# amansanghvi/Thesis

Measured on AMD Instinct MI355X. Metric: particle-updates/sec (particles x scans/s) @1081 beams, higher is better.
Workload: dtype int8 map cells (lattice log-odds), f64 poses/weights; 1 GPU; BASELINE configs[2]: room16 synthetic, 4096 particles/GPU, 1081 beams, 0.05 m grid, K=30 samples, both matcher stages, resample every step; particles_per_gpu=4096, beams=1081, parallelism=particles sharded x1

## Files before the change

thesis_amd/csrc/kernels_match.hip:

```cpp
#include <limits.h>
#include <string.h>

#include <hip/hip_ext.h>

#include "rbpf_internal.h"
#include "rbpf_device.h"

namespace rbpf {

#ifdef RBPF_STAMPS
#define MSTAMP(k) do { if (tid == 0) { long long t_ = clock64(); st_acc[k] += t_ - st_prev; st_prev = t_; } } while (0)
#else
#define MSTAMP(k) do { } while (0)
#endif

static const int MBLOCK = 512;
static const int M_COARSE = 4;
static const int M_FINE_T = 4;
static const int M_FINE_R = 4;

struct MatchArgs {
    int mode;
    int single;
    const double* ref_xy; int n_ref;
    double guess[3]; double range[3];
    double* out;
    int N;
    int ds;
    double mcs;
    double d0;
    double rot_range;
    double max_range;
    const float* sel_x; const float* sel_y; int n_sel;
    int n_coarse_rot;
    int cap_sel;
    int sc_cap;
    double cell_off;
    int ndt;
    int ndt_nc;
    int ndt_max_iter;
    const int32_t* dup_of;
    uint32_t* ndt_occ;
    double* ndt_aux;
};

struct __attribute__((packed, aligned(4))) MaskPair { uint32_t lo, hi; };
struct __attribute__((packed, aligned(4))) MaskTriple { uint32_t w0, w1, w2; };

struct MatchLds {
    uint32_t* occ;
    uint32_t* dil;
    uint32_t* crs;
    float* fx4; float* fy4;
    float* cx8; float* cy8;
    int* sc;
};

__host__ __device__ inline int match_crs_words(int N) { return ((N / M_COARSE) + 15) / 16; }
static const int CRS_PAD = 7;
// ... 44 lines not shown
    double gx, gy, gth, rx, ry;
    if (a.single) {
        gx = a.guess[0]; gy = a.guess[1]; gth = a.guess[2]; rx = a.range[0]; ry = a.range[1];
    } else {
        gx = pose5[0]; gy = pose5[1]; gth = pose5[2];
        double c00 = pose5[3], c11 = pose5[4];
        double p0 = sqrt(c00) * 30.0, p1 = sqrt(c11) * 30.0;
        ry = fmax(fmin(4 * p1, 0.7), 0.1);
        rx = fmax(fmin(4 * p0, 0.7), 0.1);
    }
    g[0] = gx; g[1] = gy; g[2] = gth; rng[0] = rx; rng[1] = ry;
    org[0] = (int)floor(gx / a.mcs) - a.N / 2;
    org[1] = (int)floor(gy / a.mcs) - a.N / 2;
}

__device__ inline void match_frame(const DevView& v, const MatchArgs& a, int p, double* g, double* rng, int* org) {
    double pose5[5] = {0, 0, 0, 0, 0};
    if (!a.single) { pose5[0] = v.px[p]; pose5[1] = v.py[p]; pose5[2] = v.pth[p]; pose5[3] = v.cov[p]; pose5[4] = v.cov[(size_t)4 * v.P + p]; }
    match_frame_from(a, pose5, g, rng, org);
}

__global__ __launch_bounds__(MBLOCK) void match_kernel(DevView v, MatchArgs a) {
    extern __shared__ __align__(16) unsigned char smem[];
    const int N = a.N, W = N >> 5, tid = threadIdx.x, p = blockIdx.x;
    const int dup = a.dup_of ? a.dup_of[p] : p;
    double pre[5] = {0, 0, 0, 0, 0}; int pre_slot = 0;
    if (!a.single && tid == 0) { pre[0] = v.px[p]; pre[1] = v.py[p]; pre[2] = v.pth[p]; pre[3] = v.cov[p]; pre[4] = v.cov[(size_t)4 * v.P + p]; }
    if (!a.single) pre_slot = v.slot[p];
    if (dup != p) { if (tid == 0) atomicAdd(&v.stats[ST_MATCH_SHARED], 1ull); return; }
    MatchLds s;
    s.occ = reinterpret_cast<uint32_t*>(smem);
    s.dil = s.occ + (size_t)N * W;
    s.crs = s.dil + (size_t)N * W;
    const int cap4 = ((a.cap_sel + 3) / 4 + 7) & ~3, cap8 = ((a.cap_sel + 7) / 8 + 7) & ~3;
    s.fx4 = reinterpret_cast<float*>(s.crs + match_crs_total(N)); s.fy4 = s.fx4 + cap4;
    s.cx8 = s.fy4 + cap4; s.cy8 = s.cx8 + cap8;
    s.sc = reinterpret_cast<int*>(s.cy8 + cap8);
    __shared__ double s_g[3], s_rng[2];
    __shared__ int s_org[2], s_nb, s_best;
    __shared__ unsigned long long s_bestc;
    __shared__ unsigned s_def[32], s_slowg;
    __shared__ double s_mom[10], s_wmom[MBLOCK / 64][10];
    __shared__ int s_tab[49];

#ifdef RBPF_STAMPS
    long long st_acc[8] = {0, 0, 0, 0, 0, 0, 0, 0}, st_prev = clock64();
#endif
// ... 606 lines not shown
    const double A10 = m[5], A20 = m[6], A21 = m[8];
    if (!(A00 > 0)) return false;
    const double l00 = sqrt(A00), l10 = A10 / l00, l20 = A20 / l00;
    const double d1 = A11 - l10 * l10;
    if (!(d1 > 0)) return false;
    const double l11 = sqrt(d1), l21 = (A21 - l20 * l10) / l11;
    const double d2 = A22 - l20 * l20 - l21 * l21;
    if (!(d2 > 0)) return false;
    const double l22 = sqrt(d2);
    const double y0 = -m[1] / l00, y1 = (-m[2] - l10 * y0) / l11, y2 = (-m[3] - l20 * y0 - l21 * y1) / l22;
    d[2] = y2 / l22;
    d[1] = (y1 - l21 * d[2]) / l11;
    d[0] = (y0 - l10 * d[1] - l20 * d[2]) / l00;
    return true;
}

static const int NBLOCK = 256;
static const int NDT_STRIDE = 1;

size_t ndt_lds_bytes(int N, int B) { (void)B; return (size_t)(N + 2) * (N / 32 + 2) * 4 + 64; }

__global__ __launch_bounds__(NBLOCK, 4) void ndt_kernel(DevView v, MatchArgs a) {
    extern __shared__ __align__(16) unsigned char smem[];
    const int N = a.N, W = N >> 5, tid = threadIdx.x, p = blockIdx.x;
    uint32_t* occ = reinterpret_cast<uint32_t*>(smem);
    const float* __restrict__ bx = a.sel_x;
    const float* __restrict__ by = a.sel_y;
    const float inv = (float)(1.0 / a.mcs);
    __shared__ double s_g[3], s_rng[2], s_trial[6], s_w[NBLOCK / 64][10];
    __shared__ int s_org[2], s_go;
    __shared__ float s_lut[5][16];
    __shared__ unsigned s_ok;
#ifdef RBPF_STAMPS
    long long st_acc[8] = {0, 0, 0, 0, 0, 0, 0, 0}, st_prev = clock64();
#endif
    if (a.dup_of && a.dup_of[p] != p) return;
    const double* aux = a.ndt_aux + (size_t)p * 5;
    if (aux[4] == 0.0 || a.n_sel <= 0) return;
    if (tid == 0) { match_frame(v, a, p, s_g, s_rng, s_org); s_ok = 0; }
    const int WPD = W + 2;
    {
        const uint32_t* src = a.ndt_occ + (size_t)p * N * W;
        int u = tid / W, wv = tid % W;
        const int du = NBLOCK / W, dw = NBLOCK % W;
        const int SL = 16;
        for (int i0 = tid; i0 < N * W; i0 += SL * NBLOCK) {
            uint32_t val[SL]; int dst[SL];
// ... 164 lines not shown
    return (2 * n_coarse_rot + 1) * (2 * k + 1) * (2 * k + 1);
}
int match_per_rot(double max_range_m, double mcs) {
    int k = (int)ceil(max_range_m / mcs / M_COARSE);
    return (2 * k + 1) * (2 * k + 1);
}

__global__ void native_sincosf_kernel(const float* x, int n, float* s, float* c) {
    const int i = blockIdx.x * blockDim.x + threadIdx.x;
    if (i >= n) return;
    float sn, cs;
    __sincosf(x[i], &sn, &cs);
    s[i] = sn; c[i] = cs;
}
void launch_native_sincosf(const float* d_x, int n, float* d_s, float* d_c, hipStream_t s) {
    if (n > 0) hipLaunchKernelGGL(native_sincosf_kernel, dim3((n + 255) / 256), dim3(256), 0, s, d_x, n, d_s, d_c);
}

static void launch_match(const DevView& v, const MatchArgs& a_in, int grid, size_t lds, hipStream_t s, hipEvent_t t0 = nullptr, hipEvent_t t1 = nullptr) {
    MatchArgs a = a_in;
    a.sc_cap = match_sc_capacity(a.N, a.cap_sel, lds);
    static size_t lds_set[MAX_DEVICES] = {};
    ensure_dynamic_lds(reinterpret_cast<const void*>(match_kernel), lds, lds_set);
    if (t0 && t1) hipExtLaunchKernelGGL(match_kernel, dim3(grid), dim3(MBLOCK), lds, s, t0, t1, 0, v, a);
    else hipLaunchKernelGGL(match_kernel, dim3(grid), dim3(MBLOCK), lds, s, v, a);
}

int ndt_cells(double mcs) { return (int)floor(0.1 / mcs + 0.5); }

static void launch_ndt(const DevView& v, const MatchArgs& a, int grid, hipStream_t s, hipEvent_t t0 = nullptr, hipEvent_t t1 = nullptr) {
    size_t lds = ndt_lds_bytes(a.N, a.cap_sel);
    static size_t lds_set[MAX_DEVICES] = {};
    ensure_dynamic_lds(reinterpret_cast<const void*>(ndt_kernel), lds, lds_set);
    if (t0 && t1) hipExtLaunchKernelGGL(ndt_kernel, dim3(grid), dim3(NBLOCK), lds, s, t0, t1, 0, v, a);
    else hipLaunchKernelGGL(ndt_kernel, dim3(grid), dim3(NBLOCK), lds, s, v, a);
}

bool launch_match_particles(const DevView& v, int mode, const double* d_ref, int n_ref, double* d_out, int N, int ds,
                            double mcs, double d0, int ncr, double max_range, int cap_sel, size_t lds, int stage, hipStream_t s,
                            hipEvent_t t0, hipEvent_t t1) {
    MatchArgs a;
    memset(&a, 0, sizeof(a));
    a.mode = mode; a.single = 0; a.ref_xy = d_ref; a.n_ref = n_ref; a.out = d_out;
    a.N = N; a.ds = ds; a.mcs = mcs; a.d0 = d0; a.rot_range = 3.141592653589793 / 6; a.max_range = max_range;
    a.sel_x = mode ? v.asel_x : v.msel_x; a.sel_y = mode ? v.asel_y : v.msel_y; a.n_sel = mode ? v.n_asel : v.n_msel;
    a.n_coarse_rot = ncr; a.cap_sel = cap_sel;
    a.ndt = v.ndt_refine; a.ndt_nc = ndt_cells(mcs); a.ndt_max_iter = 500;
    a.dup_of = v.dups_valid ? v.dup_of : nullptr;
    const bool ndt = a.ndt && a.ndt_nc >= 2 && v.ndt_occ;
    if (ndt) { a.ndt_occ = v.ndt_occ; a.ndt_aux = v.ndt_aux; }
    if (stage == 1) launch_match(v, a, v.P, lds, s, t0, t1);
    if (stage == 2 && ndt) launch_ndt(v, a, v.P, s, t0, t1);
    return ndt;
}

void launch_match_single(const DevView& v, const double* d_ref, int n_ref, const double* guess3, const double* range3,
                         const float* d_sel_x, const float* d_sel_y, int n_sel, double* d_out, int N, int ds, double mcs,
                         double d0, int ncr, int cap_sel, size_t lds, uint32_t* d_ndt_occ, double* d_ndt_aux, hipStream_t s) {
    MatchArgs a;
    memset(&a, 0, sizeof(a));
    a.mode = 1; a.single = 1; a.ref_xy = d_ref; a.n_ref = n_ref; a.out = d_out;
    for (int i = 0; i < 3; ++i) { a.guess[i] = guess3[i]; a.range[i] = range3[i]; }
    a.N = N; a.ds = ds; a.mcs = mcs; a.d0 = d0; a.rot_range = range3[2]; a.max_range = 15.0;
    a.sel_x = d_sel_x; a.sel_y = d_sel_y; a.n_sel = n_sel; a.n_coarse_rot = ncr; a.cap_sel = cap_sel;
    a.cell_off = 0.5;
    a.ndt = v.ndt_refine; a.ndt_nc = ndt_cells(mcs); a.ndt_max_iter = 500;
    const bool ndt = a.ndt && a.ndt_nc >= 2 && d_ndt_occ;
    if (ndt) { a.ndt_occ = d_ndt_occ; a.ndt_aux = d_ndt_aux; }
    launch_match(v, a, 1, lds, s);
    if (ndt) launch_ndt(v, a, 1, s);
}

}
```

thesis_amd/csrc/kernels_propose.hip:

```cpp
#include "rbpf_internal.h"
#include "rbpf_device.h"

namespace rbpf {

#ifdef RBPF_STAMPS
#define PSTAMP(k) do { if (threadIdx.x == 0) { long long t_ = clock64(); atomicAdd(&v.stats[8 + (k)], (unsigned long long)(t_ - st_prev)); st_prev = t_; } } while (0)
#else
#define PSTAMP(k) do { } while (0)
#endif


static const int KMAX = 32;

__device__ __forceinline__ void philox_round(uint32_t c[4], uint32_t k0, uint32_t k1) {
    const uint64_t p0 = (uint64_t)0xD2511F53u * c[0], p1 = (uint64_t)0xCD9E8D57u * c[2];
    uint32_t n0 = (uint32_t)(p1 >> 32) ^ c[1] ^ k0, n1 = (uint32_t)p1;
    uint32_t n2 = (uint32_t)(p0 >> 32) ^ c[3] ^ k1, n3 = (uint32_t)p0;
    c[0] = n0; c[1] = n1; c[2] = n2; c[3] = n3;
}
__device__ void philox4x32(uint32_t ctr[4], uint64_t seed) {
    uint32_t k0 = (uint32_t)seed, k1 = (uint32_t)(seed >> 32);
#pragma unroll
    for (int r = 0; r < 10; ++r) { philox_round(ctr, k0, k1); k0 += 0x9E3779B9u; k1 += 0xBB67AE85u; }
}
// ... 27 lines not shown
                    double akp = a[k][p], akq = a[k][q];
                    a[k][p] = c * akp - s * akq; a[k][q] = s * akp + c * akq;
                }
                for (int k = 0; k < 3; ++k) {
                    double apk = a[p][k], aqk = a[q][k];
                    a[p][k] = c * apk - s * aqk; a[q][k] = s * apk + c * aqk;
                }
                for (int k = 0; k < 3; ++k) {
                    double vkp = V[k][p], vkq = V[k][q];
                    V[k][p] = c * vkp - s * vkq; V[k][q] = s * vkp + c * vkq;
                }
            }
    }
    for (int i = 0; i < 3; ++i) w[i] = a[i][i];
}

struct ProposeArgs {
    const double* match;
    const int32_t* match_of;
    const double* guesses;
    uint8_t* bad;
    uint64_t seed; uint32_t stream;
    double* dbg_w;
};


static const int PREP_W = 24;
__global__ __launch_bounds__(64) void propose_prep_kernel(DevView v, ProposeArgs a) {
    const int p = blockIdx.x * 64 + threadIdx.x;
    if (p >= v.P) return;
    const double* m = a.match + (size_t)(a.match_of ? a.match_of[p] : p) * 13;
    double* o = v.prop_prep + (size_t)p * PREP_W;
    bool bad = false;
    for (int i = 0; i < 9; ++i) bad |= isnan(m[3 + i]);
    a.bad[p] = bad ? 1 : 0;
    o[22] = bad ? 1.0 : 0.0;
    if (bad) return;
    double w[3], V[3][3];
    eig3_sym(m + 3, w, V);
    double mx = fmax(fabs(w[0]), fmax(fabs(w[1]), fabs(w[2])));
    double eps = 1e6 * 2.220446049250313e-16 * mx;
    double log_pdet = 0.0; int rank = 0;
    for (int j = 0; j < 3; ++j) {
        bool keep = w[j] > eps;
        if (!keep && fabs(w[j]) > eps) { a.bad[p] = 1; o[22] = 1.0; return; }
        double inv_sqrt = fabs(w[j]) > eps ? sqrt(1.0 / w[j]) : 0.0;
        if (keep) { log_pdet += log(w[j]); ++rank; }
        double sq = w[j] > 0 ? sqrt(w[j]) : 0.0;
        for (int i = 0; i < 3; ++i) { o[3 * i + j] = V[i][j] * inv_sqrt; o[9 + 3 * i + j] = V[i][j] * sq; }
    }
    o[18] = m[0]; o[19] = m[1]; o[20] = m[2];
    o[21] = -0.5 * ((double)rank * 1.8378770664093453 + log_pdet);
}

static const int SAMP_W = 256;
__global__ __launch_bounds__(256) void propose_samples_kernel(DevView v, ProposeArgs a) {
    const int gid = blockIdx.x * 256 + threadIdx.x, p = gid >> 5, k = gid & 31, K = v.K;
    if (p >= v.P || k >= K) return;
    const double* pr = v.prop_prep + (size_t)p * PREP_W;
    if (pr[22] != 0.0) return;
    const double mean[3] = {pr[18], pr[19], pr[20]};
    double g[3];
    if (a.guesses) {
        const double* gp = a.guesses + ((size_t)p * K + k) * 3;
        g[0] = gp[0]; g[1] = gp[1]; g[2] = gp[2];
    } else {
        double z[3];
        normals3(a.seed, a.stream, (uint32_t)v.global_id[p], (uint32_t)k, z);
        for (int i = 0; i < 3; ++i) g[i] = mean[i] + ((pr[9 + 3 * i] * z[0] + pr[9 + 3 * i + 1] * z[1]) + pr[9 + 3 * i + 2] * z[2]);
    }
    const double d0 = g[0] - mean[0], d1 = g[1] - mean[1], d2 = g[2] - mean[2];
    double maha = 0.0;
    for (int j = 0; j < 3; ++j) { double t = (d0 * pr[j] + d1 * pr[3 + j]) + d2 * pr[6 + j]; maha += t * t; }
    double sn, cs;
    sincos(g[2], &sn, &cs);
    int lx, ly, off_x = 0, off_y = 0;
    if (!(v.dim & 1) && tile_of_coord(mean[0], v.tile_len, v.R, lx) && tile_of_coord(mean[1], v.tile_len, v.R, ly)) {
        off_x = v.dim / 2 - lx * v.dim; off_y = v.dim / 2 - ly * v.dim;
    }
    const double inv_cs = (double)v.dim / v.tile_len;
    double* o = v.prop_samp + (size_t)p * SAMP_W;
// ... 98 lines not shown
    for (int i = tid; i < n_redo; i += BLOCK) {
        const uint32_t e = f.s_redo[i];
        const int b = (int)(e >> 5), kk = (int)(e & 31u);
        const double x = v.bx[b], y = v.by[b];
        const double gx = (s_c[kk] * x + (-s_s[kk]) * y) + s_g[kk][0];
        const double gy = (s_s[kk] * x + s_c[kk] * y) + s_g[kk][1];
        int vv;
        if (lookup_cell_home(v, home, s_tab, s_base, gx, gy, vv)) atomicAdd(&s_sum[kk], vv);
    }
    PSTAMP(3);
}

__global__ __launch_bounds__(BLOCK) void propose_weight_kernel(DevView v, ProposeArgs a) {
    __shared__ double s_c[KMAX], s_s[KMAX], s_g[KMAX][3], s_pr[KMAX], s_w[KMAX];
    __shared__ int s_sum[KMAX];
    __shared__ float4 s_q[KMAX];
    __shared__ int s_tab[49];
    __shared__ unsigned long long s_base[49];
    __shared__ double s_mean[3];
    __shared__ double s_mom[16];
    __shared__ int s_bad, s_nredo[2];
    __shared__ uint32_t s_redo[REDO_CAP];
    __shared__ __align__(16) float s_bx[WB_CAP], s_by[WB_CAP];
    const int p = blockIdx.x, tid = threadIdx.x, K = v.K;
    long long st_prev = clock64();
    if (tid == 0) { s_nredo[0] = 0; s_nredo[1] = 0; }
    const int LL = v.L * v.L;
    {
        const double* pr = v.prop_prep + (size_t)p * PREP_W;
        if (tid < 3) s_mean[tid] = pr[18 + tid];
        if (tid == 0) s_bad = pr[22] != 0.0;
    }
    const int32_t* tab = v.tile_tab + (size_t)v.slot[p] * LL;
    for (int i = tid; i < LL; i += BLOCK) {
        const int t = tab[i];
        s_tab[i] = t;
        s_base[i] = t >= 0 ? (unsigned long long)t * (unsigned long long)v.dim * (unsigned long long)v.dim : ~0ull;
    }
    __syncthreads();
    if (s_bad) {
        if (tid == 0) { v.upd_pose[p] = v.px[p]; v.upd_pose[v.P + p] = v.py[p]; v.upd_pose[2 * v.P + p] = v.pth[p]; }
        return;
    }
    const HomeTile home = home_tile(v, s_tab, s_mean[0], s_mean[1]);
    if (tid < K) {
        const double* sp = v.prop_samp + (size_t)p * SAMP_W;
        s_c[tid] = sp[tid]; s_s[tid] = sp[32 + tid]; s_g[tid][0] = sp[64 + tid]; s_g[tid][1] = sp[96 + tid]; s_g[tid][2] = sp[128 + tid];
// ... 81 lines not shown
        s_sum[tid] = 0;
    }
    __syncthreads();
    {
        const WeightFrame wf{s_c, s_s, s_g, s_q, s_sum, s_tab, s_base, s_redo, s_nredo, s_bx, s_by};
        weight_beams(v, home, wf, K, tid, st_prev);
    }
    __syncthreads();
    if (tid < K) {
        double obs = v.inv_quantum > 0 ? (v.inv_quantum + (double)s_sum[tid]) / v.inv_quantum : 1.0 + (double)s_sum[tid] * v.quantum;
        out_w[(size_t)p * K + tid] = obs * prs[(size_t)p * K + tid];
    }
}
void launch_weight_samples_product(const DevView& v, const double* d_guesses, const double* d_prs, int K, double* d_out_w, hipStream_t s) {
    hipLaunchKernelGGL(weight_samples_product_kernel, dim3(v.P), dim3(BLOCK), 0, s, v, d_guesses, d_prs, K, d_out_w);
}

__global__ __launch_bounds__(BLOCK) void bad_weight_kernel(DevView v, const uint8_t* __restrict__ bad) {
    if (!bad[blockIdx.x]) return;
    nan_branch_weight(v, blockIdx.x, threadIdx.x, BLOCK);
}

void launch_propose_weight(const DevView& v, const double* d_match, const int32_t* d_match_of, const double* d_guesses, uint8_t* d_bad,
                           uint64_t seed, uint32_t stream, double* d_dbg_w, hipStream_t s) {
    ProposeArgs a{d_match, d_match_of, d_guesses, d_bad, seed, stream, d_dbg_w};
    hipLaunchKernelGGL(propose_prep_kernel, dim3((v.P + 63) / 64), dim3(64), 0, s, v, a);
    hipLaunchKernelGGL(propose_samples_kernel, dim3((v.P * 32 + 255) / 256), dim3(256), 0, s, v, a);
    hipLaunchKernelGGL(propose_weight_kernel, dim3(v.P), dim3(BLOCK), 0, s, v, a);
}
void launch_bad_weight(const DevView& v, const uint8_t* d_bad, hipStream_t s) {
    hipLaunchKernelGGL(bad_weight_kernel, dim3(v.P), dim3(BLOCK), 0, s, v, d_bad);
}

}
```

thesis_amd/csrc/rbpf_api.hip:

```cpp
#include <math.h>
#include <stdio.h>
#include <stdlib.h>
#include <string.h>

#include <algorithm>
#include <initializer_list>
#include <limits>

#include "rbpf_host.h"
#include "rbpf_scanbatch.h"

using namespace rbpf;

static thread_local std::string g_create_err;

#define HIP_TRY(h, call)                                                                           \
    do {                                                                                           \
        hipError_t e_ = (call);                                                                    \
        if (e_ != hipSuccess) {                                                                    \
            (h)->err = std::string(#call) + ": " + hipGetErrorString(e_);                          \
            return RBPF_EDEVICE;                                                                   \
        }                                                                                          \
    } while (0)

// ... 33 lines not shown
    if (e != hipSuccess) { h->err = std::string("hipMalloc: ") + hipGetErrorString(e); return RBPF_ENOMEM; }
    *out = h->allocs.back().as<T>();
    return RBPF_OK;
}
#define ALLOC(h, ptr, n) do { int rc_ = dev_alloc(h, &(ptr), (n)); if (rc_) return rc_; } while (0)

static int check_device_error(rbpf_handle* h) {
    int32_t e = 0;
    HIP_TRY(h, hipMemcpyAsync(&e, h->v.err, sizeof(e), hipMemcpyDeviceToHost, h->stream));
    HIP_TRY(h, hipStreamSynchronize(h->stream));
    if (e != 0) {
        int32_t z = 0;
        hipMemcpyAsync(h->v.err, &z, sizeof(z), hipMemcpyHostToDevice, h->stream);
        hipStreamSynchronize(h->stream);
        const char* what = e == RBPF_ENOMEM ? "tile pool or work-item queue exhausted"
                         : e == RBPF_ERANGE ? "a pose or beam left the addressable tile lattice (raise lattice_radius)"
                         : "device-side error";
        return fail(h, e, what);
    }
    return RBPF_OK;
}

static bool env_is(const char* name, const char* value) { const char* e = getenv(name); return e && strcmp(e, value) == 0; }

static int track_take_place(rbpf_handle* h, bool implicit, int& t) {
    t = -1;
    if (h->track_n >= h->track_cap) {
        if (!implicit) return fail(h, RBPF_ENOMEM, "the trajectory log is full");
        h->track_dropped++;
        return RBPF_OK;
    }
    t = h->track_n++;
    return RBPF_OK;
}
static int track_queue(rbpf_handle* h, int t) {
    if (t < 0) return RBPF_OK;
    launch_track_record(h->v, h->track_log(), t, h->track_pending(h->track_cur), h->stream);
    HIP_TRY(h, hipGetLastError());
    return RBPF_OK;
}
static int track_record(rbpf_handle* h, bool implicit) {
    int t;
    const int rc = track_take_place(h, implicit, t);
    return rc ? rc : track_queue(h, t);
}

// ... 159 lines not shown
        ALLOC(h, v.prop_samp, 256 * P);
        ALLOC(h, v.stats, ST_COUNT); ALLOC(h, v.err, 1);
        ALLOC(h, v.mu_fallback, P); HIP_TRY(h, hipMemset(v.mu_fallback, 0, P * 4));
        ALLOC(h, v.ev_queue, 2); HIP_TRY(h, hipMemset(v.ev_queue, 0, 8));
        ALLOC(h, h->d_did_early, 1);
        HIP_TRY(h, hipMemset(h->d_did_early, 0, 4));
        HIP_TRY(h, h->events.create(&h->ev_weights, hipEventDisableTiming | hipEventDisableSystemFence));
        {
            v.mu_mode = env_is("RBPF_MAP_KERNEL", "window") ? MU_WINDOW : env_is("RBPF_MAP_KERNEL", "ray") ? MU_RAY : env_is("RBPF_MAP_KERNEL", "ev") ? MU_EV : MU_DEFAULT;
            v.ev_resident = env_is("RBPF_EV_RESIDENT", "0") ? 0 : 1;
            const char* eg = getenv("RBPF_EV_GRID");
            v.ev_grid = eg ? std::max(0, atoi(eg)) : 0;
            v.match_stage_slow = env_is("RBPF_MATCH_STAGE", "slow") ? 1 : 0;
            const char* ws = getenv("RBPF_WSAFE");
            v.wsafe_override = ws ? (float)atof(ws) : -1.0f;
            v.weight_entry_f64 = env_is("RBPF_WEIGHT_ENTRY", "f64") ? 1 : 0;
            v.ndt_refine = h->cfg.ndt_refine;
            h->dedup_enabled = !env_is("RBPF_MATCH_DEDUP", "0");
            {
                int cus = 0;
                if (hipDeviceGetAttribute(&cus, hipDeviceAttributeMultiprocessorCount, c.device) != hipSuccess || cus < 1) { (void)hipGetLastError(); cus = 1; }
                h->skip_discarded = !env_is("RBPF_SKIP_DISCARDED", "0");
                h->hold_back = getenv("RBPF_SKIP_DISCARDED") ? true : (long long)P > 4LL * cus;
            }
        }
        ALLOC(h, v.dup_of, P); v.dups_valid = 0;
        ALLOC(h, h->d_last_xy, 2 * (size_t)c.max_beams); ALLOC(h, h->d_tmp_sel, 2 * (size_t)c.max_beams);
        if (raycast_lds_bytes(c.max_beams, v.reach) > LDS_LIMIT) return fail(h, RBPF_EINVAL, "max_beams too large for the LDS window layout");
        match_geometry(c, c.cell_size, h->mN, h->mds, h->mmcs, h->md0, h->mncr);
        h->mlds = match_lds_bytes(h->mN, c.max_beams, match_max_coarse(h->mncr, 0.7, h->mmcs), match_per_rot(0.7, h->mmcs));
        if (h->mlds > LDS_LIMIT) return fail(h, RBPF_EINVAL, "matcher region does not fit in LDS for this cell_size");
        if (c.ndt_refine && ndt_cells(h->mmcs) >= 2) {
            if (ndt_lds_bytes(h->mN, c.max_beams) > LDS_LIMIT) return fail(h, RBPF_EINVAL, "NDT stage: matcher region does not fit in LDS");
            ALLOC(h, v.ndt_occ, P * (size_t)h->mN * (h->mN / 32)); ALLOC(h, v.ndt_aux, 5 * P);
        }
        ALLOC(h, h->d_match, 13 * P); ALLOC(h, h->d_bad, P); ALLOC(h, h->d_guess_full, P * (size_t)c.n_samples * 3);
        {
            ResampleBuffers& r = h->rs;
            ALLOC(h, r.T, P); ALLOC(h, r.idx, P); ALLOC(h, r.did, 1); ALLOC(h, r.slot2, P); ALLOC(h, r.dead_list, P);
            ALLOC(h, r.jobs, 2 * P); ALLOC(h, r.n_jobs, 2); ALLOC(h, r.pending_free, (size_t)v.pool_tiles); ALLOC(h, r.n_pending, 1);
            ALLOC(h, r.px2, P); ALLOC(h, r.py2, P); ALLOC(h, r.pth2, P); ALLOC(h, r.cov2, 9 * P); ALLOC(h, r.w2, P);
            ALLOC(h, r.skip, P); ALLOC(h, r.keep, P); ALLOC(h, r.plan, 2);
            HIP_TRY(h, hipMemset(r.n_pending, 0, 4)); HIP_TRY(h, hipMemset(r.n_jobs, 0, 8)); HIP_TRY(h, hipMemset(r.did, 0, 4));
            HIP_TRY(h, hipMemset(r.skip, 0, P)); HIP_TRY(h, hipMemset(r.plan, 0, 8));
        }
        HIP_TRY(h, hipMemset(v.pool, 0, (size_t)v.pool_tiles * cells));
// ... 6 lines not shown
        for (size_t p = 0; p < P; ++p) { ids[p] = (int32_t)p; tab[p * LL + (size_t)v.R * v.L + v.R] = (int32_t)p; }
        for (int t = 0; t < v.pool_tiles; ++t) { bb[4 * t] = INT32_MAX; bb[4 * t + 1] = -1; bb[4 * t + 2] = INT32_MAX; bb[4 * t + 3] = -1; }
        int32_t top = v.pool_tiles - (int32_t)P;
        for (int i = 0; i < top; ++i) fs[i] = v.pool_tiles - 1 - i;
        HIP_TRY(h, hipMemcpy(v.slot, ids.data(), P * 4, hipMemcpyHostToDevice));
        HIP_TRY(h, hipMemcpy(v.global_id, ids.data(), P * 4, hipMemcpyHostToDevice));
        HIP_TRY(h, hipMemcpy(v.tile_tab, tab.data(), P * LL * 4, hipMemcpyHostToDevice));
        HIP_TRY(h, hipMemcpy(v.free_stack, fs.data(), (size_t)v.pool_tiles * 4, hipMemcpyHostToDevice));
        HIP_TRY(h, hipMemcpy(v.free_top, &top, 4, hipMemcpyHostToDevice));
        HIP_TRY(h, hipMemcpy(v.tile_bbox, bb.data(), bb.size() * 4, hipMemcpyHostToDevice));
        return RBPF_OK;
    };
    rc = build();
    if (rc != RBPF_OK) { g_create_err = h->err; rbpf_destroy(h); return rc; }
    *out = h;
    return RBPF_OK;
}

int rbpf_destroy(rbpf_handle* h) {
    if (!h) return RBPF_OK;
    ON_DEVICE_HELD(h);
    h->mu_pending = false;
    if (hipStreamSynchronize(h->stream) != hipSuccess) (void)hipGetLastError();
    h->each_staging([](Staging& s) { if (s.wait() != hipSuccess) (void)hipGetLastError(); });
    if (h->ev_weights_valid && hipEventSynchronize(h->ev_weights) != hipSuccess) (void)hipGetLastError();
    for (Block& b : h->allocs) b.release();
    for (Block& b : h->buf) b.release();
    for (Block& b : h->track_mem) b.release();
    h->each_staging([](Staging& s) { s.release(); });
    h->each_staging([](Staging& s) { s.destroy_event(); });
    h->events.destroy();
    if (h->own_stream && h->stream) (void)hipStreamDestroy(h->stream);
    (void)hipGetLastError();
    delete h;
    return RBPF_OK;
}

const char* rbpf_last_error(const rbpf_handle* h) { return h ? h->err.c_str() : g_create_err.c_str(); }

int rbpf_set_stream(rbpf_handle* h, void* s) {
    if (!h) return RBPF_EINVAL;
    ON_DEVICE(h);
    HIP_TRY(h, hipStreamSynchronize(h->stream));
    if (h->own_stream && h->stream) (void)hipStreamDestroy(h->stream);
    h->own_stream = false;
    h->stream = static_cast<hipStream_t>(s);
    h->last_end = nullptr;
    return RBPF_OK;
}

int rbpf_release_stream(rbpf_handle* h) {
    if (!h) return RBPF_EINVAL;
    ON_DEVICE(h);
    if (h->own_stream) return RBPF_OK;
    HIP_TRY(h, hipStreamSynchronize(h->stream));
// ... 205 lines not shown
int rbpf_map_update(rbpf_handle* h, const double* poses) {
    if (!h) return RBPF_EINVAL;
    ON_DEVICE(h);
    h->v.dups_valid = 0;
    if (!h->have_scan) return fail(h, RBPF_ESTATE, "rbpf_set_scan has not been called");
    DevView& v = h->v;
    const size_t P = v.P;
    if (poses) {
        std::vector<double> soa(3 * P);
        for (size_t p = 0; p < P; ++p) { soa[p] = poses[3 * p]; soa[P + p] = poses[3 * p + 1]; soa[2 * P + p] = poses[3 * p + 2]; }
        HIP_TRY(h, hipMemcpyAsync(v.upd_pose, soa.data(), 3 * P * 8, hipMemcpyHostToDevice, h->stream));
        HIP_TRY(h, hipStreamSynchronize(h->stream));
    } else {
        HIP_TRY(h, hipMemcpyAsync(v.upd_pose, v.px, P * 8, hipMemcpyDeviceToDevice, h->stream));
        HIP_TRY(h, hipMemcpyAsync(v.upd_pose + P, v.py, P * 8, hipMemcpyDeviceToDevice, h->stream));
        HIP_TRY(h, hipMemcpyAsync(v.upd_pose + 2 * P, v.pth, P * 8, hipMemcpyDeviceToDevice, h->stream));
    }
    int rc = run_map_update(h, h->v);
    if (rc) return rc;
    h->scan_updates++;
    return check_device_error(h);
}

static int run_matcher(rbpf_handle* h, int32_t adj, const double* last_scan_xy, int32_t n_last) {
    DevView& v = h->v;
    if (adj && !last_scan_xy) {
        if (h->n_last_dev < 0) return fail(h, RBPF_ESTATE, "adj = 1 without last_scan_xy needs rbpf_refresh_last_scan first");
        n_last = h->n_last_dev;
    } else if (adj && (n_last < 0 || n_last > h->cfg.max_beams))
        return fail(h, RBPF_EINVAL, "adj = 1 needs last_scan_xy with at most max_beams points");
    if (adj && last_scan_xy) {
        void* slot = h->rings[R_LAST].acquire();
        memcpy(slot, last_scan_xy, (size_t)n_last * 16);
        HIP_TRY(h, hipMemcpyAsync(h->d_last_xy, slot, (size_t)n_last * 16, hipMemcpyHostToDevice, h->stream));
        h->rings[R_LAST].submitted(h->stream);
    }
    hipEvent_t t0 = nullptr, t1 = nullptr;
    h->prof_take(3, t0, t1);
    h->match_rows = v.dups_valid ? 2 : 1;
    const bool ndt = launch_match_particles(v, adj ? 1 : 0, h->d_last_xy, adj ? n_last : 0, h->d_match, h->mN, h->mds, h->mmcs, h->md0,
                                            h->mncr, h->cfg.match_max_range, h->cfg.max_beams, h->mlds, 1, h->stream, t0, t1);
    if (ndt) {
        h->prof_take(4, t0, t1);
        launch_match_particles(v, adj ? 1 : 0, h->d_last_xy, adj ? n_last : 0, h->d_match, h->mN, h->mds, h->mmcs, h->md0,
                               h->mncr, h->cfg.match_max_range, h->cfg.max_beams, h->mlds, 2, h->stream, t0, t1);
    }
    HIP_TRY(h, hipGetLastError());
    return RBPF_OK;
}

int rbpf_scan_update(rbpf_handle* h, int32_t adj, const double* last_scan_xy, int32_t n_last,
                     const double* match_override, const double* guesses) {
    int rc = rbpf_scan_update_begin(h, adj, last_scan_xy, n_last, match_override, guesses);
    if (rc || !h->map_updates || !h->hold_back) return rc ? rc : rbpf_scan_update_end(h);
    h->scan_begun = false;
    h->scan_updates++;
    h->mu_pending = true; h->mu_pending_rec = -1;
    if (h->track_on && (h->track_flags & RBPF_TRACK_SCAN)) return track_take_place(h, true, h->mu_pending_rec);
    return RBPF_OK;
}

int rbpf_scan_update_begin(rbpf_handle* h, int32_t adj, const double* last_scan_xy, int32_t n_last,
                           const double* match_override, const double* guesses) {
    if (!h) return RBPF_EINVAL;
    ON_DEVICE(h);
    if (!h->have_scan) return fail(h, RBPF_ESTATE, "rbpf_set_scan has not been called");
    DevView& v = h->v;
    const size_t P = v.P;
    if (match_override) {
        h->match_rows = 0;
        HIP_TRY(h, hipMemcpyAsync(h->d_match, match_override, 13 * P * 8, hipMemcpyHostToDevice, h->stream));
    } else {
        int rc = run_matcher(h, adj, last_scan_xy, n_last);
        if (rc) return rc;
    }
    const double* d_g = nullptr;
    if (guesses) {
        HIP_TRY(h, hipMemcpyAsync(h->d_guess_full, guesses, P * (size_t)v.K * 3 * 8, hipMemcpyHostToDevice, h->stream));
        d_g = h->d_guess_full;
    }
    if (!match_override && !guesses) h->prof_begin_chained(1); else h->prof_begin(1);
    const int32_t* match_of = (!match_override && v.dups_valid) ? v.dup_of : nullptr;
    if (h->prop_capture && !h->d_prop_w) ALLOC(h, h->d_prop_w, P * (size_t)v.K);
    launch_propose_weight(v, h->d_match, match_of, d_g, h->d_bad, h->cfg.seed, (uint32_t)h->scan_updates, h->prop_capture ? h->d_prop_w : nullptr, h->stream);
    h->prop_valid = true; h->prop_captured = h->prop_capture;
    v.dups_valid = 0;
    h->prof_end(1);
    HIP_TRY(h, hipGetLastError());
    h->ev_weights_valid = false;
    if (h->record_ev_weights) { HIP_TRY(h, hipEventRecord(h->ev_weights, h->stream)); h->ev_weights_valid = true; }
    h->scan_begun = true; h->begin_seen = true;
    return RBPF_OK;
}

int rbpf_scan_update_end(rbpf_handle* h) {
    if (!h) return RBPF_EINVAL;
    ON_DEVICE(h);
    if (!h->scan_begun) return fail(h, RBPF_ESTATE, "rbpf_scan_update_begin has not been called");
    h->scan_begun = false;
    if (!h->map_updates) {
        launch_bad_weight(h->v, h->d_bad, h->stream);
        HIP_TRY(h, hipGetLastError());
        h->scan_updates++;
    } else {
        const int rc = run_map_update(h, h->v, h->d_bad);
        if (rc) return rc;
        h->scan_updates++;
    }
    if (h->track_on && (h->track_flags & RBPF_TRACK_SCAN)) return track_record(h, true);
    return RBPF_OK;
// ... 2176 lines not shown
```

thesis_amd/csrc/rbpf_host.h:

```cpp
#pragma once
#include <stdlib.h>
#include <algorithm>
#include <string>
#include <vector>

#include "rbpf_internal.h"

static const size_t LDS_LIMIT = 160 * 1024;

enum MemKind { MEM_DEVICE, MEM_PINNED, MEM_PAGEABLE };
struct Block {
    MemKind kind = MEM_DEVICE;
    unsigned char* p = nullptr; size_t cap = 0;
    hipError_t reserve(size_t bytes) {
        if (p && cap >= bytes) return hipSuccess;
        release();
        const size_t want = kind == MEM_PINNED ? std::max<size_t>(bytes * 2, 1 << 16) : std::max<size_t>(bytes, 4096);
        hipError_t e = hipSuccess;
        if (kind == MEM_DEVICE) e = hipMalloc(reinterpret_cast<void**>(&p), want);
        else if (kind == MEM_PINNED) e = hipHostMalloc(reinterpret_cast<void**>(&p), want, hipHostMallocDefault);
        else if (!(p = static_cast<unsigned char*>(malloc(want)))) e = hipErrorOutOfMemory;
        if (e == hipSuccess) cap = want; else p = nullptr;
        return e;
    }
// ... 115 lines not shown
    hipError_t reserve(int b, size_t bytes) {
        if (buf[b].cap >= bytes) return hipSuccess;
        if (b >= B_DRAIN_FIRST) { const hipError_t e = hipStreamSynchronize(stream); if (e != hipSuccess) return e; }
        return buf[b].reserve(bytes);
    }
    PinnedRing rings[R_COUNT];
    EventPool events;
    template <typename F> void each_staging(F f) { for (Staging& s : stage) f(s); for (PinnedRing& r : rings) for (Staging& s : r.slot) f(s); }
    hipEvent_t ev_weights = nullptr; bool ev_weights_valid = false, record_ev_weights = false, begin_seen = false;
    int32_t* d_did_early = nullptr; bool scan_begun = false;
    int early_n = 0;
    unsigned char* d_scan = nullptr; size_t scan_bytes = 0;
    template <typename T> T* in_slot(unsigned char* slot, const T* dev) const { return reinterpret_cast<T*>(slot + (reinterpret_cast<const unsigned char*>(dev) - d_scan)); }
    int mN = 0, mds = 1, mncr = 0; double mmcs = 0, md0 = 0; size_t mlds = 0;
    double* d_last_xy = nullptr; float* d_tmp_sel = nullptr;
    int n_last_dev = -1;
    int match_rows = 0;
    double* d_match = nullptr; uint8_t* d_bad = nullptr; double* d_guess_full = nullptr;
    unsigned long long resample_draws = 0;
    int ev_workgroups = 0;
    bool map_updates = true;
    bool mu_pending = false; int mu_pending_rec = -1;
    bool hold_back = false, skip_discarded = true;
    static const int N_KERN = 5, RING = 512;
    std::vector<hipEvent_t> ring[N_KERN][2];
    int ring_n[N_KERN] = {0, 0, 0, 0, 0};
    std::vector<hipEvent_t> begin_used[N_KERN];
    hipEvent_t last_end = nullptr;
    bool timed(int k) const { return (prof_mask >> k) & 1u; }
    void prof_begin(int k) { if (!timed(k)) return; hipEvent_t e = ring[k][0][ring_n[k] % RING]; (void)hipEventRecord(e, stream); begin_used[k][ring_n[k] % RING] = e; if (k == 2) rs_split[ring_n[k] % RING] = 0; }
    void prof_begin_chained(int k) { if (!timed(k)) return; if (!last_end) { prof_begin(k); return; } begin_used[k][ring_n[k] % RING] = last_end; }
    void prof_end(int k) { if (!timed(k)) return; last_end = ring[k][1][ring_n[k] % RING]; (void)hipEventRecord(last_end, stream); ring_n[k]++; }
    std::vector<hipEvent_t> rs_mid[2]; std::vector<char> rs_split;
    void prof_pause(int k) { if (!timed(k)) return; const int slot = ring_n[k] % RING; (void)hipEventRecord(rs_mid[0][slot], stream); rs_split[slot] = 1; }
    void prof_resume(int k) { if (!timed(k)) return; (void)hipEventRecord(rs_mid[1][ring_n[k] % RING], stream); }
    hipError_t family_ms(int k, int slot, float* ms) {
        if (k != 2 || !rs_split[slot]) return hipEventElapsedTime(ms, begin_used[k][slot], ring[k][1][slot]);
        float a = 0, b = 0;
        hipError_t e = hipEventElapsedTime(&a, begin_used[k][slot], rs_mid[0][slot]);
        if (e == hipSuccess) e = hipEventElapsedTime(&b, rs_mid[1][slot], ring[k][1][slot]);
        *ms = a + b;
        return e;
    }
    bool prof_take(int k, hipEvent_t& t0, hipEvent_t& t1) {
        t0 = t1 = nullptr;
        if (!timed(k)) return false;
// ... 19 lines not shown
```

thesis_amd/csrc/rbpf_internal.h:

```cpp
#pragma once
#include <hip/hip_runtime.h>
#include <stdint.h>
#include <mutex>

#include "../../include/rbpf_hip.h"
#include "rbpf_math.h"
#include "rbpf_blockrelax.h"

namespace rbpf {

static const int MAX_DEVICES = 16;
inline void ensure_dynamic_lds(const void* fn, size_t bytes, size_t* set) {
    static std::mutex mu;
    std::lock_guard<std::mutex> lock(mu);
    int dev = 0;
    (void)hipGetDevice(&dev);
    const bool tracked = dev >= 0 && dev < MAX_DEVICES;
    if (tracked && bytes <= set[dev]) return;
    const hipError_t rc = hipFuncSetAttribute(fn, hipFuncAttributeMaxDynamicSharedMemorySize, (int)bytes);
    if (rc != hipSuccess) { (void)hipGetLastError(); return; }
    if (tracked) set[dev] = bytes;
}


// ... 323 lines not shown
void launch_readback(void* mapped_dst, const double* d_nan_elem, const int32_t* d_did, const int32_t* d_idx, int n, hipStream_t s);
bool map_update_ray_available(const DevView& v);
void launch_map_update_ray(const DevView& v, const int32_t* only, hipStream_t s, hipEvent_t t0 = nullptr, hipEvent_t t1 = nullptr);
bool map_update_ev_available(const DevView& v);
int launch_map_update_ev(const DevView& v, hipStream_t s, hipEvent_t t0 = nullptr, hipEvent_t t1 = nullptr);
void launch_get_odds(const DevView& v, int particle, const double* d_xy, int n, double* d_vals,
                     uint8_t* d_none, hipStream_t s);
void launch_last_scan(const DevView& v, int particle, double* d_out_xy, hipStream_t s);
void launch_imu_update(const DevView& v, int model, double d0, double d1, double d2, double dt_ticks,
                       const double* vel_noise, hipStream_t s);
void launch_resample_indices(int P, const double* d_w, double u, double spread, int32_t* d_T, int32_t* d_idx,
                             int32_t* d_did, int32_t* d_err, hipStream_t s);
void launch_resample_local(const DevView& v, const ResampleBuffers& b, const double* d_w, double u, double spread, hipStream_t s);
void launch_resample_plan_early(const DevView& v, const ResampleBuffers& b, const uint8_t* d_bad, int leave_out, double u, double spread, hipStream_t s);
void launch_resample_plan_late(const DevView& v, const ResampleBuffers& b, double u, double spread, hipStream_t s);
void launch_resample_copies(const DevView& v, const ResampleBuffers& b, hipStream_t s);
void launch_export_weights(const DevView& v, double* d_out, int n_global, const uint8_t* d_bad, hipStream_t s);
void launch_gather_meta(const DevView& v, const int32_t* d_local, int n, int32_t* d_out, hipStream_t s);
void launch_pack(const DevView& v, const void* d_jobs, int n_jobs, void* d_buf, hipStream_t s);
void launch_unpack(const DevView& v, const ResampleBuffers& b, const void* d_jobs, int n_jobs, const void* d_buf, hipStream_t s);
struct PackJobHost { int32_t particle, tile, x0, x1, ya, yb; long long off; };
struct UnpackJobHost { int32_t particle, pos, has, x0, x1, ya, yb, pad; long long off; };
void launch_propose_weight(const DevView& v, const double* d_match, const int32_t* d_match_of, const double* d_guesses, uint8_t* d_bad,
                           uint64_t seed, uint32_t stream, double* d_dbg_w, hipStream_t s);
void launch_bad_weight(const DevView& v, const uint8_t* d_bad, hipStream_t s);
size_t match_lds_bytes(int N, int B, int n_coarse, int per_rot);
int match_sc_capacity(int N, int B, size_t lds);
int match_per_rot(double max_range_m, double mcs);
size_t ndt_lds_bytes(int N, int B);
int ndt_cells(double mcs);
void match_geometry(const rbpf_config& c, double cell_size, int& N, int& ds, double& mcs, double& d0, int& n_coarse_rot);
int match_max_coarse(int n_coarse_rot, double max_range_m, double mcs);
bool launch_match_particles(const DevView& v, int mode, const double* d_ref, int n_ref, double* d_out, int N, int ds,
                            double mcs, double d0, int ncr, double max_range, int cap_sel, size_t lds, int stage, hipStream_t s,
                            hipEvent_t t0 = nullptr, hipEvent_t t1 = nullptr);
void launch_match_single(const DevView& v, const double* d_ref, int n_ref, const double* guess3, const double* range3,
                         const float* d_sel_x, const float* d_sel_y, int n_sel, double* d_out, int N, int ds, double mcs,
                         double d0, int ncr, int cap_sel, size_t lds, uint32_t* d_ndt_occ, double* d_ndt_aux, hipStream_t s);
void launch_match_inputs(const DevView& v, int particle, const double* guess3, double* d_all_curr, int* d_counts,
                         uint32_t* d_mask, int* d_row_cnt, double* d_ref, int cap_ref, double* d_curr, int win,
                         double match_max, hipStream_t s);
void launch_native_sincosf(const float* d_x, int n, float* d_s, float* d_c, hipStream_t s);
size_t raycast_lds_bytes(int B, int reach);
void launch_map_extent(const DevView& v, int particle, int32_t* d_box4, hipStream_t s);
void launch_render_cells(const DevView& v, int particle, const RenderJob* d_jobs, int n_jobs, long long ny, int8_t* d_out,
                         hipStream_t s);
void launch_render_filter(const DevView& v, const RenderFilter& f, int n_jobs, int G, hipStream_t s);
void launch_load_validate(const DevView& v, const LoadArgs& a, hipStream_t s);
void launch_load_map(const DevView& v, const LoadArgs& a, int n_jobs, hipStream_t s);
void launch_load_alloc(const DevView& v, const LoadArgs& a, hipStream_t s);
void launch_place_warp(const PlaceArgs& q, hipStream_t s);
void launch_place_map(const DevView& v, const LoadArgs& a, const PlaceArgs& q, int n_jobs, hipStream_t s);
void launch_cast_scans(const DevView& v, const CastArgs& a, hipStream_t s);
size_t view_gain_lds_bytes(int M, int W);
void launch_view_gain(const DevView& v, const GainArgs& a, hipStream_t s);
void launch_build_map(const BuildArgs& a, hipStream_t s);
size_t refine_lds_bytes(int Mw, int WW);
void launch_refine_poses(const DevView& v, const LocateArgs& f, const RefineArgs& a, hipStream_t s);
// ... 19 lines not shown
```

Before: 2.357 million particle-updates/s.

## Split particles into two chunks so matching overlaps proposal weighting across streams

Adds a particle offset and count to the match, NDT and propose kernels. When the particle count per CU falls in a mid range, the front end runs as two chunks. The first chunk's match, NDT and propose/weight run on a high-priority side stream while the main stream matches the second chunk. Events gate the second chunk's weighting on the first chunk's match results, because duplicate-of indices may point into the first chunk. The aim is to fill the GPU tail and idle gaps between the match stage and the weight stage. The cost is extra launches, event synchronisation, and possible contention between the concurrent kernels.

```diff
diff --git a/thesis_amd/csrc/kernels_match.hip b/thesis_amd/csrc/kernels_match.hip
--- a/thesis_amd/csrc/kernels_match.hip
+++ b/thesis_amd/csrc/kernels_match.hip
@@ -35,6 +35,7 @@
     int n_coarse_rot;
     int cap_sel;
     int sc_cap;
+    int p0;
     double cell_off;
     int ndt;
     int ndt_nc;
@@ -125,7 +126,7 @@
 
 __global__ __launch_bounds__(MBLOCK) void match_kernel(DevView v, MatchArgs a) {
     extern __shared__ __align__(16) unsigned char smem[];
-    const int N = a.N, W = N >> 5, tid = threadIdx.x, p = blockIdx.x;
+    const int N = a.N, W = N >> 5, tid = threadIdx.x, p = a.p0 + blockIdx.x;
     const int dup = a.dup_of ? a.dup_of[p] : p;
     double pre[5] = {0, 0, 0, 0, 0}; int pre_slot = 0;
     if (!a.single && tid == 0) { pre[0] = v.px[p]; pre[1] = v.py[p]; pre[2] = v.pth[p]; pre[3] = v.cov[p]; pre[4] = v.cov[(size_t)4 * v.P + p]; }
@@ -778,7 +779,7 @@
 
 __global__ __launch_bounds__(NBLOCK, 4) void ndt_kernel(DevView v, MatchArgs a) {
     extern __shared__ __align__(16) unsigned char smem[];
-    const int N = a.N, W = N >> 5, tid = threadIdx.x, p = blockIdx.x;
+    const int N = a.N, W = N >> 5, tid = threadIdx.x, p = a.p0 + blockIdx.x;
     uint32_t* occ = reinterpret_cast<uint32_t*>(smem);
     const float* __restrict__ bx = a.sel_x;
     const float* __restrict__ by = a.sel_y;
@@ -989,7 +990,7 @@
     a.sc_cap = match_sc_capacity(a.N, a.cap_sel, lds);
     static size_t lds_set[MAX_DEVICES] = {};
     ensure_dynamic_lds(reinterpret_cast<const void*>(match_kernel), lds, lds_set);
-    if (t0 && t1) hipExtLaunchKernelGGL(match_kernel, dim3(grid), dim3(MBLOCK), lds, s, t0, t1, 0, v, a);
+    if (t0 || t1) hipExtLaunchKernelGGL(match_kernel, dim3(grid), dim3(MBLOCK), lds, s, t0, t1, 0, v, a);
     else hipLaunchKernelGGL(match_kernel, dim3(grid), dim3(MBLOCK), lds, s, v, a);
 }
 
@@ -999,25 +1000,26 @@
     size_t lds = ndt_lds_bytes(a.N, a.cap_sel);
     static size_t lds_set[MAX_DEVICES] = {};
     ensure_dynamic_lds(reinterpret_cast<const void*>(ndt_kernel), lds, lds_set);
-    if (t0 && t1) hipExtLaunchKernelGGL(ndt_kernel, dim3(grid), dim3(NBLOCK), lds, s, t0, t1, 0, v, a);
+    if (t0 || t1) hipExtLaunchKernelGGL(ndt_kernel, dim3(grid), dim3(NBLOCK), lds, s, t0, t1, 0, v, a);
     else hipLaunchKernelGGL(ndt_kernel, dim3(grid), dim3(NBLOCK), lds, s, v, a);
 }
 
 bool launch_match_particles(const DevView& v, int mode, const double* d_ref, int n_ref, double* d_out, int N, int ds,
-                            double mcs, double d0, int ncr, double max_range, int cap_sel, size_t lds, int stage, hipStream_t s,
-                            hipEvent_t t0, hipEvent_t t1) {
+                            double mcs, double d0, int ncr, double max_range, int cap_sel, size_t lds, int stage, int p0, int n,
+                            hipStream_t s, hipEvent_t t0, hipEvent_t t1) {
     MatchArgs a;
     memset(&a, 0, sizeof(a));
     a.mode = mode; a.single = 0; a.ref_xy = d_ref; a.n_ref = n_ref; a.out = d_out;
     a.N = N; a.ds = ds; a.mcs = mcs; a.d0 = d0; a.rot_range = 3.141592653589793 / 6; a.max_range = max_range;
     a.sel_x = mode ? v.asel_x : v.msel_x; a.sel_y = mode ? v.asel_y : v.msel_y; a.n_sel = mode ? v.n_asel : v.n_msel;
-    a.n_coarse_rot = ncr; a.cap_sel = cap_sel;
+    a.n_coarse_rot = ncr; a.cap_sel = cap_sel; a.p0 = p0;
     a.ndt = v.ndt_refine; a.ndt_nc = ndt_cells(mcs); a.ndt_max_iter = 500;
     a.dup_of = v.dups_valid ? v.dup_of : nullptr;
     const bool ndt = a.ndt && a.ndt_nc >= 2 && v.ndt_occ;
     if (ndt) { a.ndt_occ = v.ndt_occ; a.ndt_aux = v.ndt_aux; }
-    if (stage == 1) launch_match(v, a, v.P, lds, s, t0, t1);
-    if (stage == 2 && ndt) launch_ndt(v, a, v.P, s, t0, t1);
+    if (n <= 0) return ndt;
+    if (stage == 1) launch_match(v, a, n, lds, s, t0, t1);
+    if (stage == 2 && ndt) launch_ndt(v, a, n, s, t0, t1);
     return ndt;
 }
 
diff --git a/thesis_amd/csrc/kernels_propose.hip b/thesis_amd/csrc/kernels_propose.hip
--- a/thesis_amd/csrc/kernels_propose.hip
+++ b/thesis_amd/csrc/kernels_propose.hip
@@ -1,3 +1,5 @@
+#include <hip/hip_ext.h>
+
 #include "rbpf_internal.h"
 #include "rbpf_device.h"
 
@@ -73,13 +75,14 @@
     uint8_t* bad;
     uint64_t seed; uint32_t stream;
     double* dbg_w;
+    int p0, n;
 };
 
 
 static const int PREP_W = 24;
 __global__ __launch_bounds__(64) void propose_prep_kernel(DevView v, ProposeArgs a) {
-    const int p = blockIdx.x * 64 + threadIdx.x;
-    if (p >= v.P) return;
+    const int i = blockIdx.x * 64 + threadIdx.x, p = a.p0 + i;
+    if (i >= a.n) return;
     const double* m = a.match + (size_t)(a.match_of ? a.match_of[p] : p) * 13;
     double* o = v.prop_prep + (size_t)p * PREP_W;
     bool bad = false;
@@ -106,8 +109,8 @@
 
 static const int SAMP_W = 256;
 __global__ __launch_bounds__(256) void propose_samples_kernel(DevView v, ProposeArgs a) {
-    const int gid = blockIdx.x * 256 + threadIdx.x, p = gid >> 5, k = gid & 31, K = v.K;
-    if (p >= v.P || k >= K) return;
+    const int gid = blockIdx.x * 256 + threadIdx.x, p = a.p0 + (gid >> 5), k = gid & 31, K = v.K;
+    if ((gid >> 5) >= a.n || k >= K) return;
     const double* pr = v.prop_prep + (size_t)p * PREP_W;
     if (pr[22] != 0.0) return;
     const double mean[3] = {pr[18], pr[19], pr[20]};
@@ -252,7 +255,7 @@
     __shared__ int s_bad, s_nredo[2];
     __shared__ uint32_t s_redo[REDO_CAP];
     __shared__ __align__(16) float s_bx[WB_CAP], s_by[WB_CAP];
-    const int p = blockIdx.x, tid = threadIdx.x, K = v.K;
+    const int p = a.p0 + blockIdx.x, tid = threadIdx.x, K = v.K;
     long long st_prev = clock64();
     if (tid == 0) { s_nredo[0] = 0; s_nredo[1] = 0; }
     const int LL = v.L * v.L;
@@ -380,11 +383,13 @@
 }
 
 void launch_propose_weight(const DevView& v, const double* d_match, const int32_t* d_match_of, const double* d_guesses, uint8_t* d_bad,
-                           uint64_t seed, uint32_t stream, double* d_dbg_w, hipStream_t s) {
-    ProposeArgs a{d_match, d_match_of, d_guesses, d_bad, seed, stream, d_dbg_w};
-    hipLaunchKernelGGL(propose_prep_kernel, dim3((v.P + 63) / 64), dim3(64), 0, s, v, a);
-    hipLaunchKernelGGL(propose_samples_kernel, dim3((v.P * 32 + 255) / 256), dim3(256), 0, s, v, a);
-    hipLaunchKernelGGL(propose_weight_kernel, dim3(v.P), dim3(BLOCK), 0, s, v, a);
+                           uint64_t seed, uint32_t stream, double* d_dbg_w, int p0, int n, hipStream_t s, hipEvent_t done) {
+    if (n <= 0) return;
+    ProposeArgs a{d_match, d_match_of, d_guesses, d_bad, seed, stream, d_dbg_w, p0, n};
+    hipLaunchKernelGGL(propose_prep_kernel, dim3((n + 63) / 64), dim3(64), 0, s, v, a);
+    hipLaunchKernelGGL(propose_samples_kernel, dim3((n * 32 + 255) / 256), dim3(256), 0, s, v, a);
+    if (done) hipExtLaunchKernelGGL(propose_weight_kernel, dim3(n), dim3(BLOCK), 0, s, nullptr, done, 0, v, a);
+    else hipLaunchKernelGGL(propose_weight_kernel, dim3(n), dim3(BLOCK), 0, s, v, a);
 }
 void launch_bad_weight(const DevView& v, const uint8_t* d_bad, hipStream_t s) {
     hipLaunchKernelGGL(bad_weight_kernel, dim3(v.P), dim3(BLOCK), 0, s, v, d_bad);
diff --git a/thesis_amd/csrc/rbpf_api.hip b/thesis_amd/csrc/rbpf_api.hip
--- a/thesis_amd/csrc/rbpf_api.hip
+++ b/thesis_amd/csrc/rbpf_api.hip
@@ -79,6 +79,7 @@
 }
 
 static bool env_is(const char* name, const char* value) { const char* e = getenv(name); return e && strcmp(e, value) == 0; }
+static const long long SCAN_HALVES_MIN_PER_CU = 12, SCAN_HALVES_END_PER_CU = 20;
 
 static int track_take_place(rbpf_handle* h, bool implicit, int& t) {
     t = -1;
@@ -284,6 +285,16 @@
                 if (hipDeviceGetAttribute(&cus, hipDeviceAttributeMultiprocessorCount, c.device) != hipSuccess || cus < 1) { (void)hipGetLastError(); cus = 1; }
                 h->skip_discarded = !env_is("RBPF_SKIP_DISCARDED", "0");
                 h->hold_back = getenv("RBPF_SKIP_DISCARDED") ? true : (long long)P > 4LL * cus;
+                const bool halves = env_is("RBPF_SCAN_HALVES", "0") ? false : getenv("RBPF_SCAN_HALVES") ? true : ((long long)P >= SCAN_HALVES_MIN_PER_CU * cus && (long long)P < SCAN_HALVES_END_PER_CU * cus);
+                if (halves) {
+                    int least = 0, greatest = 0;
+                    HIP_TRY(h, hipDeviceGetStreamPriorityRange(&least, &greatest));
+                    HIP_TRY(h, hipStreamCreateWithPriority(&h->side, hipStreamNonBlocking, greatest));
+                    HIP_TRY(h, h->events.create(&h->ev_fork, hipEventDisableTiming | hipEventDisableSystemFence));
+                    HIP_TRY(h, h->events.create(&h->ev_half_match, hipEventDisableSystemFence));
+                    HIP_TRY(h, h->events.create(&h->ev_half_weight, hipEventDisableSystemFence));
+                    h->halves_first = (int)(P - std::max<size_t>(P > 1 ? 1 : 0, 3 * P / 8));
+                }
             }
         }
         ALLOC(h, v.dup_of, P); v.dups_valid = 0;
@@ -336,6 +347,7 @@
     ON_DEVICE_HELD(h);
     h->mu_pending = false;
     if (hipStreamSynchronize(h->stream) != hipSuccess) (void)hipGetLastError();
+    if (h->side && hipStreamSynchronize(h->side) != hipSuccess) (void)hipGetLastError();
     h->each_staging([](Staging& s) { if (s.wait() != hipSuccess) (void)hipGetLastError(); });
     if (h->ev_weights_valid && hipEventSynchronize(h->ev_weights) != hipSuccess) (void)hipGetLastError();
     for (Block& b : h->allocs) b.release();
@@ -345,6 +357,7 @@
     h->each_staging([](Staging& s) { s.destroy_event(); });
     h->events.destroy();
     if (h->own_stream && h->stream) (void)hipStreamDestroy(h->stream);
+    if (h->side) (void)hipStreamDestroy(h->side);
     (void)hipGetLastError();
     delete h;
     return RBPF_OK;
@@ -596,8 +609,7 @@
     return check_device_error(h);
 }
 
-static int run_matcher(rbpf_handle* h, int32_t adj, const double* last_scan_xy, int32_t n_last) {
-    DevView& v = h->v;
+static int stage_last_scan(rbpf_handle* h, int32_t adj, const double* last_scan_xy, int32_t& n_last) {
     if (adj && !last_scan_xy) {
         if (h->n_last_dev < 0) return fail(h, RBPF_ESTATE, "adj = 1 without last_scan_xy needs rbpf_refresh_last_scan first");
         n_last = h->n_last_dev;
@@ -609,16 +621,43 @@
         HIP_TRY(h, hipMemcpyAsync(h->d_last_xy, slot, (size_t)n_last * 16, hipMemcpyHostToDevice, h->stream));
         h->rings[R_LAST].submitted(h->stream);
     }
+    return RBPF_OK;
+}
+
+static bool match_stage(rbpf_handle* h, int32_t adj, int32_t n_last, int stage, int p0, int n, hipStream_t s, hipEvent_t t0 = nullptr, hipEvent_t t1 = nullptr) {
+    return launch_match_particles(h->v, adj ? 1 : 0, h->d_last_xy, adj ? n_last : 0, h->d_match, h->mN, h->mds, h->mmcs, h->md0,
+                                  h->mncr, h->cfg.match_max_range, h->cfg.max_beams, h->mlds, stage, p0, n, s, t0, t1);
+}
+
+static int run_matcher(rbpf_handle* h, int32_t adj, int32_t n_last) {
     hipEvent_t t0 = nullptr, t1 = nullptr;
     h->prof_take(3, t0, t1);
-    h->match_rows = v.dups_valid ? 2 : 1;
-    const bool ndt = launch_match_particles(v, adj ? 1 : 0, h->d_last_xy, adj ? n_last : 0, h->d_match, h->mN, h->mds, h->mmcs, h->md0,
-                                            h->mncr, h->cfg.match_max_range, h->cfg.max_beams, h->mlds, 1, h->stream, t0, t1);
-    if (ndt) {
+    if (match_stage(h, adj, n_last, 1, 0, h->v.P, h->stream, t0, t1)) {
         h->prof_take(4, t0, t1);
-        launch_match_particles(v, adj ? 1 : 0, h->d_last_xy, adj ? n_last : 0, h->d_match, h->mN, h->mds, h->mmcs, h->md0,
-                               h->mncr, h->cfg.match_max_range, h->cfg.max_beams, h->mlds, 2, h->stream, t0, t1);
-    }
+        match_stage(h, adj, n_last, 2, 0, h->v.P, h->stream, t0, t1);
+    }
+    HIP_TRY(h, hipGetLastError());
+    return RBPF_OK;
+}
+
+static int run_front_halves(rbpf_handle* h, int32_t adj, int32_t n_last, const int32_t* match_of, const double* d_g) {
+    const DevView& v = h->v;
+    const int n0 = std::min(h->halves_first, v.P), n1 = v.P - n0;
+    const bool ndt = match_stage(h, adj, n_last, 0, 0, 0, h->stream);
+    double* dbg = h->prop_capture ? h->d_prop_w : nullptr;
+    HIP_TRY(h, hipEventRecord(h->ev_fork, h->stream));
+    HIP_TRY(h, hipStreamWaitEvent(h->side, h->ev_fork, 0));
+    match_stage(h, adj, n_last, 1, 0, n0, h->side, nullptr, ndt || !n1 ? nullptr : h->ev_half_match);
+    if (ndt) match_stage(h, adj, n_last, 2, 0, n0, h->side, nullptr, n1 ? h->ev_half_match : nullptr);
+    launch_propose_weight(v, h->d_match, match_of, d_g, h->d_bad, h->cfg.seed, (uint32_t)h->scan_updates, dbg, 0, n0, h->side, h->ev_half_weight);
+    HIP_TRY(h, hipGetLastError());
+    if (n1) {
+        match_stage(h, adj, n_last, 1, n0, n1, h->stream);
+        if (ndt) match_stage(h, adj, n_last, 2, n0, n1, h->stream);
+        HIP_TRY(h, hipStreamWaitEvent(h->stream, h->ev_half_match, 0));
+        launch_propose_weight(v, h->d_match, match_of, d_g, h->d_bad, h->cfg.seed, (uint32_t)h->scan_updates, dbg, n0, n1, h->stream);
+    }
+    HIP_TRY(h, hipStreamWaitEvent(h->stream, h->ev_half_weight, 0));
     HIP_TRY(h, hipGetLastError());
     return RBPF_OK;
 }
@@ -645,21 +684,28 @@
         h->match_rows = 0;
         HIP_TRY(h, hipMemcpyAsync(h->d_match, match_override, 13 * P * 8, hipMemcpyHostToDevice, h->stream));
     } else {
-        int rc = run_matcher(h, adj, last_scan_xy, n_last);
+        const int rc = stage_last_scan(h, adj, last_scan_xy, n_last);
         if (rc) return rc;
+        h->match_rows = v.dups_valid ? 2 : 1;
     }
     const double* d_g = nullptr;
     if (guesses) {
         HIP_TRY(h, hipMemcpyAsync(h->d_guess_full, guesses, P * (size_t)v.K * 3 * 8, hipMemcpyHostToDevice, h->stream));
         d_g = h->d_guess_full;
     }
-    if (!match_override && !guesses) h->prof_begin_chained(1); else h->prof_begin(1);
     const int32_t* match_of = (!match_override && v.dups_valid) ? v.dup_of : nullptr;
     if (h->prop_capture && !h->d_prop_w) ALLOC(h, h->d_prop_w, P * (size_t)v.K);
-    launch_propose_weight(v, h->d_match, match_of, d_g, h->d_bad, h->cfg.seed, (uint32_t)h->scan_updates, h->prop_capture ? h->d_prop_w : nullptr, h->stream);
+    if (!match_override && h->halves_now()) {
+        const int rc = run_front_halves(h, adj, n_last, match_of, d_g);
+        if (rc) return rc;
+    } else {
+        if (!match_override) { const int rc = run_matcher(h, adj, n_last); if (rc) return rc; }
+        if (!match_override && !guesses) h->prof_begin_chained(1); else h->prof_begin(1);
+        launch_propose_weight(v, h->d_match, match_of, d_g, h->d_bad, h->cfg.seed, (uint32_t)h->scan_updates, h->prop_capture ? h->d_prop_w : nullptr, 0, v.P, h->stream);
+        h->prof_end(1);
+    }
     h->prop_valid = true; h->prop_captured = h->prop_capture;
     v.dups_valid = 0;
-    h->prof_end(1);
     HIP_TRY(h, hipGetLastError());
     h->ev_weights_valid = false;
     if (h->record_ev_weights) { HIP_TRY(h, hipEventRecord(h->ev_weights, h->stream)); h->ev_weights_valid = true; }
diff --git a/thesis_amd/csrc/rbpf_host.h b/thesis_amd/csrc/rbpf_host.h
--- a/thesis_amd/csrc/rbpf_host.h
+++ b/thesis_amd/csrc/rbpf_host.h
@@ -161,6 +161,10 @@
     bool map_updates = true;
     bool mu_pending = false; int mu_pending_rec = -1;
     bool hold_back = false, skip_discarded = true;
+    hipStream_t side = nullptr;
+    int halves_first = 0;
+    hipEvent_t ev_fork = nullptr, ev_half_match = nullptr, ev_half_weight = nullptr;
+    bool halves_now() const { return halves_first > 0 && side && !(prof_mask & 0x1Au); }
     static const int N_KERN = 5, RING = 512;
     std::vector<hipEvent_t> ring[N_KERN][2];
     int ring_n[N_KERN] = {0, 0, 0, 0, 0};
diff --git a/thesis_amd/csrc/rbpf_internal.h b/thesis_amd/csrc/rbpf_internal.h
--- a/thesis_amd/csrc/rbpf_internal.h
+++ b/thesis_amd/csrc/rbpf_internal.h
@@ -369,7 +369,7 @@
 struct PackJobHost { int32_t particle, tile, x0, x1, ya, yb; long long off; };
 struct UnpackJobHost { int32_t particle, pos, has, x0, x1, ya, yb, pad; long long off; };
 void launch_propose_weight(const DevView& v, const double* d_match, const int32_t* d_match_of, const double* d_guesses, uint8_t* d_bad,
-                           uint64_t seed, uint32_t stream, double* d_dbg_w, hipStream_t s);
+                           uint64_t seed, uint32_t stream, double* d_dbg_w, int p0, int n, hipStream_t s, hipEvent_t done = nullptr);
 void launch_bad_weight(const DevView& v, const uint8_t* d_bad, hipStream_t s);
 size_t match_lds_bytes(int N, int B, int n_coarse, int per_rot);
 int match_sc_capacity(int N, int B, size_t lds);
@@ -379,8 +379,8 @@
 void match_geometry(const rbpf_config& c, double cell_size, int& N, int& ds, double& mcs, double& d0, int& n_coarse_rot);
 int match_max_coarse(int n_coarse_rot, double max_range_m, double mcs);
 bool launch_match_particles(const DevView& v, int mode, const double* d_ref, int n_ref, double* d_out, int N, int ds,
-                            double mcs, double d0, int ncr, double max_range, int cap_sel, size_t lds, int stage, hipStream_t s,
-                            hipEvent_t t0 = nullptr, hipEvent_t t1 = nullptr);
+                            double mcs, double d0, int ncr, double max_range, int cap_sel, size_t lds, int stage, int p0, int n,
+                            hipStream_t s, hipEvent_t t0 = nullptr, hipEvent_t t1 = nullptr);
 void launch_match_single(const DevView& v, const double* d_ref, int n_ref, const double* guess3, const double* range3,
                          const float* d_sel_x, const float* d_sel_y, int n_sel, double* d_out, int N, int ds, double mcs,
                          double d0, int ncr, int cap_sel, size_t lds, uint32_t* d_ndt_occ, double* d_ndt_aux, hipStream_t s);
```

Result: faster. 2.410 million particle-updates/s (median of 6 runs) (+2.3%).
